# srndpty/kobato-eyes

Measured on AMD Instinct MI355X. Metric: images/s (pHash + all-pairs Hamming scan + cluster membership), higher is better.
Workload: dtype u8 luma, int32 taps (i8 matrix cores), f64 DCT, 1-bit Hamming products (fp4 matrix cores, exact)

## Files before the change

### kobato-eyes_amd/csrc/ke_api.hip

```cpp
#include <cstdarg>
#include <cstdio>
#include <algorithm>
#include <cmath>
#include <numeric>
#include <unordered_map>

#include <fcntl.h>
#include <sys/stat.h>
#include <unistd.h>

#include "ke_internal.h"

static thread_local std::string g_create_err;

int ke_fail(ke_ctx *ctx, int code, const char *fmt, ...) {
    char msg[512];
    va_list ap;
    va_start(ap, fmt);
    vsnprintf(msg, sizeof msg, fmt, ap);
    va_end(ap);
    if (ctx)
        ctx->err = msg;
    else
        g_create_err = msg;
// ... 45 lines not shown
    if (bytes) KE_HIP(ctx, hipMemcpyAsync(d, p, bytes, hipMemcpyHostToDevice, ctx->stream));
    *dev = d;
    return KE_OK;
}

static int upload_i32(ke_ctx *ctx, const std::vector<int32_t> &v, int32_t **out) {
    KE_HIP(ctx, hipMalloc((void **)out, std::max<size_t>(v.size(), 4) * sizeof(int32_t)));
    if (!v.empty())
        KE_HIP(ctx, hipMemcpy(*out, v.data(), v.size() * sizeof(int32_t), hipMemcpyHostToDevice));
    return KE_OK;
}

constexpr size_t kMaxCoeffTables = 2048;

static void free_coeff_cache(ke_ctx *ctx) {
    for (auto &kv : ctx->coeffs) {
        KeAxisCoeffs *c = kv.second;
        for (int32_t *p : {c->d_bounds, c->d_kk, c->d_start, c->d_bias, c->d_packed})
            if (p) (void)hipFree(p);
        for (auto &ck : c->chunked) {
            if (ck.second->d_cstart) (void)hipFree(ck.second->d_cstart);
            if (ck.second->d_cpacked) (void)hipFree(ck.second->d_cpacked);
            if (ck.second->d_cxor) (void)hipFree(ck.second->d_cxor);
            delete ck.second;
        }
        for (auto &mk : c->mx) {
            if (mk.second->d_frag) (void)hipFree(mk.second->d_frag);
            delete mk.second;
        }
        delete c;
    }
    ctx->coeffs.clear();
}

static void trim_coeff_cache(ke_ctx *ctx) {
    if (ctx->coeffs.size() <= kMaxCoeffTables) return;
    (void)hipStreamSynchronize(ctx->stream);
    free_coeff_cache(ctx);
}

const KeAxisCoeffs *ke_get_coeffs(ke_ctx *ctx, int in_size, int out_size, int filter, float in0, float in1) {
    if (in1 < 0.0f) { in0 = 0.0f; in1 = (float)in_size; }
    uint32_t b0, b1;
    std::memcpy(&b0, &in0, 4);
    std::memcpy(&b1, &in1, 4);
    auto key = std::make_tuple(in_size, out_size * 4 + filter, b0, b1);
    auto it = ctx->coeffs.find(key);
    if (it != ctx->coeffs.end()) return it->second;
    auto *c = new KeAxisCoeffs();
    ke_build_axis_coeffs(in_size, out_size, *c, filter, in0, in1);
    if (upload_i32(ctx, c->bounds, &c->d_bounds) || upload_i32(ctx, c->kk, &c->d_kk) ||
        upload_i32(ctx, c->start, &c->d_start) || upload_i32(ctx, c->bias, &c->d_bias) ||
        upload_i32(ctx, c->packed, &c->d_packed)) {
        delete c;
        return nullptr;
    }
    ctx->coeffs[key] = c;
    return c;
}

const KeChunkTable *ke_get_chunks(ke_ctx *ctx, const KeAxisCoeffs *cc, int cpo, int ndwc_multiple) {
    auto *c = const_cast<KeAxisCoeffs *>(cc);
    const int key = cpo * 64 + ndwc_multiple;
    auto it = c->chunked.find(key);
    if (it != c->chunked.end()) return it->second;
    auto *t = new KeChunkTable();
    ke_build_chunked(*c, cpo, *t, ndwc_multiple);
    if (upload_i32(ctx, t->cstart, &t->d_cstart) || upload_i32(ctx, t->cpacked, &t->d_cpacked) ||
        upload_i32(ctx, t->cxor, &t->d_cxor)) {
        delete t;
        return nullptr;
    }
    c->chunked[key] = t;
    return t;
}

const KeMxTable *ke_get_mx(ke_ctx *ctx, const KeAxisCoeffs *cc, int min_ks, bool align64) {
    auto *c = const_cast<KeAxisCoeffs *>(cc);
    const int key = min_ks * 2 + (align64 ? 1 : 0);
    auto it = c->mx.find(key);
    if (it != c->mx.end()) return it->second;
    auto *t = new KeMxTable();
    ke_build_mx(*c, *t, min_ks, align64);
    if (upload_i32(ctx, t->frag, &t->d_frag)) {
        delete t;
        return nullptr;
    }
    c->mx[key] = t;
    return t;
}

void ke_time_begin(ke_ctx *ctx, int kind) {
    ctx->ev_valid[kind] = false;
    (void)hipEventRecord(ctx->ev0[kind], ctx->stream);
}

void ke_time_end(ke_ctx *ctx, int kind) {
    if (hipEventRecord(ctx->ev1[kind], ctx->stream) == hipSuccess) ctx->ev_valid[kind] = true;
}

KE_API int ke_abi_version(void) { return KE_ABI_VERSION; }

KE_API const char *ke_create_error(void) { return g_create_err.c_str(); }

KE_API ke_ctx *ke_create(int device_id) {
    int count = 0;
    if (hipGetDeviceCount(&count) != hipSuccess || count <= 0) {
        ke_fail(nullptr, KE_ENODEV, "no HIP device visible (libkeyes_hip has no CPU fallback)");
        return nullptr;
    }
    if (device_id < 0 || device_id >= count) {
        ke_fail(nullptr, KE_EINVAL, "device_id %d out of range [0,%d)", device_id, count);
        return nullptr;
    }
    if (hipSetDevice(device_id) != hipSuccess) {
        ke_fail(nullptr, KE_EHIP, "hipSetDevice(%d) failed", device_id);
        return nullptr;
    }
    hipDeviceProp_t prop;
    if (hipGetDeviceProperties(&prop, device_id) != hipSuccess) {
        ke_fail(nullptr, KE_EHIP, "hipGetDeviceProperties failed");
        return nullptr;
    }
    if (std::strncmp(prop.gcnArchName, "gfx950", 6) != 0) {
        ke_fail(nullptr, KE_ENODEV, "device %d is %s; this library is built for gfx950 only", device_id,
                prop.gcnArchName);
        return nullptr;
    }
    auto *ctx = new ke_ctx();
    ctx->device = device_id;
    ctx->cu_count = prop.multiProcessorCount;
    if (hipStreamCreateWithFlags(&ctx->own_stream, hipStreamNonBlocking) != hipSuccess) {
        ke_fail(nullptr, KE_EHIP, "hipStreamCreate failed");
        delete ctx;
        return nullptr;
    }
    ctx->stream = ctx->own_stream;
    for (int k = 0; k < KE_T_COUNT; ++k) {
        (void)hipEventCreate(&ctx->ev0[k]);
        (void)hipEventCreate(&ctx->ev1[k]);
    }
    return ctx;
}

static void stage_free(ke_ctx *ctx);

KE_API void ke_destroy(ke_ctx *ctx) {
    if (!ctx) return;
    (void)hipSetDevice(ctx->device);
    (void)hipStreamSynchronize(ctx->stream);
    stage_free(ctx);
    for (int k = 0; k < 2; ++k) {
        if (ctx->side[k]) (void)hipStreamDestroy(ctx->side[k]);
        if (ctx->side_join[k]) (void)hipEventDestroy(ctx->side_join[k]);
    }
    if (ctx->side_fork) (void)hipEventDestroy(ctx->side_fork);
    if (ctx->h_comm) (void)hipHostFree(ctx->h_comm);
    if (ctx->h_meta) (void)hipHostFree(ctx->h_meta);
    for (auto &b : ctx->buf)
        if (b.ptr) (void)hipFree(b.ptr);
    free_coeff_cache(ctx);
    for (int k = 0; k < KE_T_COUNT; ++k) {
        (void)hipEventDestroy(ctx->ev0[k]);
        (void)hipEventDestroy(ctx->ev1[k]);
    }
    (void)hipStreamDestroy(ctx->own_stream);
// ... 982 lines not shown
```

### kobato-eyes_amd/csrc/ke_coeffs.cpp

```cpp
#include <algorithm>
#include <cmath>

#include "ke_internal.h"

namespace {

constexpr int kPrecisionBits = 22;
constexpr double kPi = 3.14159265358979323846;

inline double sinc_pi(double x) {
    if (x == 0.0) return 1.0;
    const double a = x * kPi;
    return std::sin(a) / a;
}

inline double lanczos3(double x) {
    return (x >= -3.0 && x < 3.0) ? sinc_pi(x) * sinc_pi(x / 3.0) : 0.0;
}

inline double triangle(double x) {
    if (x < 0.0) x = -x;
    return x < 1.0 ? 1.0 - x : 0.0;
}

// ... 44 lines not shown
                const double v = total != 0.0 ? w[t] / total : w[t];
                k[t] = v < 0 ? (int32_t)(v * (double)(1 << kPrecisionBits) - 0.5)
                             : (int32_t)(v * (double)(1 << kPrecisionBits) + 0.5);
            }
            c.bounds[2 * o] = lo;
            c.bounds[2 * o + 1] = cnt;
        }
    }

    int ndw = 0;
    c.start.assign((size_t)out_size, 0);
    for (int o = 0; o < out_size; ++o) {
        const int lo = c.bounds[2 * o], cnt = c.bounds[2 * o + 1];
        const int st = lo & ~7;
        c.start[o] = st;
        const int need = (lo + cnt - st + 3) / 4;
        if (need > ndw) ndw = need;
    }
    ndw = (ndw + 3) & ~3;
    c.ndw = ndw;
    c.span = 0;
    c.bias.assign((size_t)out_size, 0);
    c.packed.assign((size_t)out_size * ndw * 3, 0);
    for (int o = 0; o < out_size; ++o) {
        const int lo = c.bounds[2 * o], cnt = c.bounds[2 * o + 1], st = c.start[o];
        if (st + 4 * ndw > c.span) c.span = st + 4 * ndw;
        int64_t ksum = 0;
        for (int j = 0; j < ndw; ++j) {
            uint32_t plane[3] = {0, 0, 0};
            for (int e = 0; e < 4; ++e) {
                const int t = st + 4 * j + e - lo;
                const int32_t k = (t >= 0 && t < cnt) ? c.kk[(size_t)o * c.ksize + t] : 0;
                ksum += k;
                const int32_t b0 = ((k + 128) & 255) - 128;
                const int32_t r1 = (k - b0) >> 8;
                const int32_t b1 = ((r1 + 128) & 255) - 128;
                const int32_t b2 = (r1 - b1) >> 8;
                plane[0] |= (uint32_t)(b0 & 255) << (8 * e);
                plane[1] |= (uint32_t)(b1 & 255) << (8 * e);
                plane[2] |= (uint32_t)(b2 & 255) << (8 * e);
            }
            for (int p = 0; p < 3; ++p) c.packed[((size_t)o * ndw + j) * 3 + p] = (int32_t)plane[p];
        }
        c.bias[o] = (int32_t)(128 * ksum + (1 << (kPrecisionBits - 1)));
    }
}

void ke_build_mx(const KeAxisCoeffs &c, KeMxTable &t, int min_ks, bool align64) {
    t.tiles = (c.out_size + 15) / 16;
    t.base.assign((size_t)t.tiles, 0);
    t.ks = std::max(1, min_ks);
    for (int j = 0; j < t.tiles; ++j) {
        int lo = c.in_size, hi = 0;
        for (int o = 16 * j; o < std::min(16 * j + 16, c.out_size); ++o) {
            lo = std::min(lo, c.bounds[2 * o]);
            hi = std::max(hi, c.bounds[2 * o] + c.bounds[2 * o + 1]);
        }
        const int ks16 = (hi - (lo & ~15) + 63) / 64, ks64 = (hi - (lo & ~63) + 63) / 64;
        t.base[j] = (align64 || ks64 == ks16) ? (lo & ~63) : (lo & ~15);
        t.ks = std::max(t.ks, align64 ? ks64 : ks16);
    }
    t.frag.assign((size_t)t.tiles * t.ks * 3 * 64 * 4, 0);
    for (int j = 0; j < t.tiles; ++j)
        for (int s = 0; s < t.ks; ++s)
            for (int l = 0; l < 64; ++l) {
                const int o = 16 * j + (l & 15);
                if (o >= c.out_size) continue;
                const int lo = c.bounds[2 * o], cnt = c.bounds[2 * o + 1];
                for (int e = 0; e < 16; ++e) {
                    const int tap = t.base[j] + 64 * s + 16 * (l >> 4) + e - lo;
                    const int32_t k = (tap >= 0 && tap < cnt) ? c.kk[(size_t)o * c.ksize + tap] : 0;
                    const int32_t b0 = ((k + 128) & 255) - 128;
                    const int32_t r1 = (k - b0) >> 8;
                    const int32_t b1 = ((r1 + 128) & 255) - 128;
                    const int32_t b2 = (r1 - b1) >> 8;
                    const int32_t plane[3] = {b0, b1, b2};
                    for (int p = 0; p < 3; ++p)
                        t.frag[((((size_t)j * t.ks + s) * 3 + p) * 64 + l) * 4 + e / 4] |=
                            (int32_t)((uint32_t)(plane[p] & 255) << (8 * (e % 4)));
                }
            }
}

void ke_build_chunked(const KeAxisCoeffs &c, int cpo, KeChunkTable &t, int ndwc_multiple) {
    t.cpo = cpo;
    t.ndwc = (((c.ndw + cpo - 1) / cpo) + ndwc_multiple - 1) / ndwc_multiple * ndwc_multiple;
    const int nv = c.out_size * cpo;
    t.cstart.assign((size_t)nv, 0);
    t.cpacked.assign((size_t)nv * t.ndwc * 3, 0);
    t.cspan = 0;
    for (int o = 0; o < c.out_size; ++o)
        for (int k = 0; k < cpo; ++k) {
            const int v = o * cpo + k;
            t.cstart[v] = c.start[o] + 4 * t.ndwc * k;
            if (t.cstart[v] + 4 * t.ndwc > t.cspan) t.cspan = t.cstart[v] + 4 * t.ndwc;
            for (int j = 0; j < t.ndwc; ++j) {
                const int src = k * t.ndwc + j;
                if (src >= c.ndw) continue;
                for (int p = 0; p < 3; ++p)
                    t.cpacked[((size_t)v * t.ndwc + j) * 3 + p] = c.packed[((size_t)o * c.ndw + src) * 3 + p];
            }
        }
    t.cxor.assign((size_t)nv, 0);
    if (t.ndwc % 8 == 0) {
        const int np = t.ndwc / 2;
        for (int g0 = 0; g0 < nv; g0 += 32) {
            for (int v = g0; v < std::min(nv, g0 + 32); ++v) {
                int best_x = 0, best_hits = 1 << 30;
                for (int x = 0; x < 4; ++x) {
                    int hits = 0;
                    for (int p = 0; p < np; ++p) {
                        const int slot = ((t.cstart[v] / 8) + (p ^ x)) & 31;
                        for (int u = g0; u < v; ++u)
                            if ((((t.cstart[u] / 8) + (p ^ t.cxor[u])) & 31) == slot) ++hits;
                    }
                    if (hits < best_hits) { best_hits = hits; best_x = x; }
                }
                t.cxor[v] = best_x;
            }
        }
    }
}
```

### kobato-eyes_amd/csrc/ke_hash.hip

```cpp
#include <cstdlib>

#include "ke_internal.h"
#include "dct_table.h"

namespace {

constexpr int kPrecisionBits = 22;

__device__ __forceinline__ int clip8_fixed(int acc) {
    int v = acc >> kPrecisionBits;
    return v < 0 ? 0 : (v > 255 ? 255 : v);
}

__device__ __forceinline__ int luma_of(const uint8_t *p, int ch) {
    if (ch == 1) return p[0];
    return (int)((19595u * p[0] + 38470u * p[1] + 7471u * p[2] + 0x8000u) >> 16);
}

template <int AXIS>
__global__ __launch_bounds__(256) void ke_resample_pass(const uint8_t *__restrict__ src,
                                                         const uint64_t *__restrict__ offsets, uint64_t stride,
                                                         int ch, int w, int h, const int32_t *__restrict__ bounds,
                                                         const int32_t *__restrict__ kk, int ksize, int out_size,
                                                         uint8_t *__restrict__ dst, int blocks_per_image) {
    const int64_t img = blockIdx.x / blocks_per_image;
    const int blk = blockIdx.x % blocks_per_image;
    const int ow = AXIS == 0 ? out_size : w;
    const int oh = AXIS == 0 ? h : out_size;
    const int e = blk * 256 + threadIdx.x;
    if (e >= ow * oh) return;
    const int oy = e / ow, ox = e % ow;
    const uint8_t *base = src + (offsets ? offsets[img] : (uint64_t)img * stride);
    const int o = AXIS == 0 ? ox : oy;
    const int first = bounds[2 * o], cnt = bounds[2 * o + 1];
    const int32_t *k = kk + (size_t)o * ksize;
    int acc = 1 << (kPrecisionBits - 1);
    if (AXIS == 0) {
        const uint8_t *row = base + ((size_t)oy * w + first) * ch;
        for (int t = 0; t < cnt; ++t) acc += luma_of(row + (size_t)t * ch, ch) * k[t];
    } else {
        const uint8_t *col = base + ((size_t)first * w + ox) * ch;
        for (int t = 0; t < cnt; ++t) acc += luma_of(col + (size_t)t * w * ch, ch) * k[t];
    }
    dst[(size_t)img * ow * oh + e] = (uint8_t)clip8_fixed(acc);
}

__constant__ double c_C32[4][16];
__constant__ double c_C16[2][8];
__constant__ double c_C8[4];

__device__ double dct32_one(const double *x, int k) {
    if (k & 1) {
        const int q = k >> 1;
        double acc = 0.0;
#pragma unroll
        for (int n = 0; n < 16; ++n) acc = fma(x[n] - x[31 - n], c_C32[q][n], acc);
        return acc;
    }
    double u[16];
#pragma unroll
    for (int n = 0; n < 16; ++n) u[n] = x[n] + x[31 - n];
    if (k & 2) {
        const int q = k >> 2;
        double acc = 0.0;
#pragma unroll
        for (int n = 0; n < 8; ++n) acc = fma(u[n] - u[15 - n], c_C16[q][n], acc);
        return acc;
    }
    double v[8];
#pragma unroll
    for (int n = 0; n < 8; ++n) v[n] = u[n] + u[15 - n];
    if (k == 4) {
        double acc = 0.0;
#pragma unroll
        for (int n = 0; n < 4; ++n) acc = fma(v[n] - v[7 - n], c_C8[n], acc);
        return acc;
    }
    const double w0 = v[0] + v[7], w1 = v[1] + v[6], w2 = v[2] + v[5], w3 = v[3] + v[4];
    return (w0 + w1) + (w2 + w3);
}

__device__ uint64_t tile32_to_phash(const uint8_t *tile, double *Td, float *cf, int tid, float *margin = nullptr) {
    {
// ... 160 lines not shown
#pragma unroll
            for (int m = 0; m < 4; ++m) {
                const uint2 v = *reinterpret_cast<const uint2 *>(
                    __builtin_assume_aligned(HT + (size_t)(og + 8 * m) * a.hp + vst + 4 * jj, 8));
                acc[m][0] = __builtin_amdgcn_sdot4((int)v.x, c00, acc[m][0], false);
                acc[m][1] = __builtin_amdgcn_sdot4((int)v.x, c01, acc[m][1], false);
                acc[m][2] = __builtin_amdgcn_sdot4((int)v.x, c02, acc[m][2], false);
                acc[m][0] = __builtin_amdgcn_sdot4((int)v.y, c10, acc[m][0], false);
                acc[m][1] = __builtin_amdgcn_sdot4((int)v.y, c11, acc[m][1], false);
                acc[m][2] = __builtin_amdgcn_sdot4((int)v.y, c12, acc[m][2], false);
            }
        }
        const int vbias = a.v_bias[yy];
#pragma unroll
        for (int m = 0; m < 4; ++m)
            T32[yy * 32 + og + 8 * m] = (uint8_t)clip8_fixed(combine_planes(acc[m][0], acc[m][1], acc[m][2], vbias));
    }
    __syncthreads();
    if (a.tile32_out)
        reinterpret_cast<uint32_t *>(a.tile32_out + (size_t)img * 1024)[tid] = reinterpret_cast<const uint32_t *>(T32)[tid];
    const int64_t slot = a.out_idx ? a.out_idx[img] : img;
    const uint64_t hv = tile32_to_phash(T32, Td, cf, tid, (a.margin && a.phash) ? a.margin + slot : nullptr);
    if (tid == 0 && a.phash) a.phash[slot] = hv;
    if (NDWD > 0) {
        __syncthreads();
        int *part = reinterpret_cast<int *>(Lt);
        uint8_t *T98 = Lt + 1024;
        if (tid < 216) {
            const int out = tid / 3, chunk = tid % 3;
            const int yy = out / 9, oc = out % 9;
            const int vc = yy * 3 + chunk;
            const int vst = a.vd_cstart[vc];
            const int nd = a.ndwcv;
            int d0 = 0, d1 = 0, d2 = 0;
            for (int j = 0; j < nd; j += 2) {
                const int32_t *cp = a.vd_cpacked + ((size_t)vc * nd + j) * 3;
                const uint2 v = *reinterpret_cast<const uint2 *>(__builtin_assume_aligned(HTd + (size_t)oc * a.hpd + vst + 4 * j, 8));
                d0 = __builtin_amdgcn_sdot4((int)v.x, cp[0], d0, false);
                d1 = __builtin_amdgcn_sdot4((int)v.x, cp[1], d1, false);
                d2 = __builtin_amdgcn_sdot4((int)v.x, cp[2], d2, false);
                d0 = __builtin_amdgcn_sdot4((int)v.y, cp[3], d0, false);
                d1 = __builtin_amdgcn_sdot4((int)v.y, cp[4], d1, false);
                d2 = __builtin_amdgcn_sdot4((int)v.y, cp[5], d2, false);
            }
            part[tid] = combine_planes(d0, d1, d2, 0);
        }
        __syncthreads();
        if (tid < 72) {
            const int yy = tid / 9;
            const uint32_t sum = (uint32_t)part[3 * tid] + (uint32_t)part[3 * tid + 1] + (uint32_t)part[3 * tid + 2] + (uint32_t)a.vd_bias[yy];
            T98[tid] = (uint8_t)clip8_fixed((int)sum);
        }
        __syncthreads();
        if (a.tile98_out && tid < 72) a.tile98_out[(size_t)img * 72 + tid] = T98[tid];
        if (tid < 64) {
            const int r = tid >> 3, c = tid & 7;
            const unsigned long long m = __ballot(T98[r * 9 + c + 1] > T98[r * 9 + c]);
            if (tid == 0 && a.dhash) a.dhash[a.out_idx ? a.out_idx[img] : img] = __brevll(m);
        }
    }
}

int upload_dct_tables(ke_ctx *ctx) {
    if (ctx->dct_tables_ready) return KE_OK;
    KE_HIP(ctx, hipMemcpyToSymbol(HIP_SYMBOL(c_C32), KE_C32, sizeof(KE_C32)));
    KE_HIP(ctx, hipMemcpyToSymbol(HIP_SYMBOL(c_C16), KE_C16, sizeof(KE_C16)));
    KE_HIP(ctx, hipMemcpyToSymbol(HIP_SYMBOL(c_C8), KE_C8, sizeof(KE_C8)));
    ctx->dct_tables_ready = true;
    return KE_OK;
}

constexpr int kRTM = 32;
typedef int ke_v4i __attribute__((ext_vector_type(4)));

template <int W64, int KS, bool DH, bool GEN, int C, bool UNAL>
__global__ __launch_bounds__(256, 2) void ke_phash_fused_mx(const KeFusedArgs a) {
    static_assert(!UNAL || GEN, "rows that are not a multiple of 4 pixels need the run-time row length");
    constexpr uint32_t QB = 4u * C;
    constexpr int W = 64 * W64;
    constexpr int QPT = kRTM * (W / 4) / 256;
    const int QW = GEN ? a.qw : W / 4;
    const int QUADS_PER_TILE = kRTM * QW;
    const int LP = GEN ? a.lp : W + 16;
    constexpr int KD = (W64 + 1) / 2;
    extern __shared__ __attribute__((aligned(16))) uint8_t smem[];
    uint8_t *Lt = smem;
    uint8_t *HT = smem + a.lt_bytes;
    uint8_t *HTd = HT + 32 * a.hp;
    uint8_t *X = smem + a.x_off;
    const int tid = threadIdx.x;
    const int lane = tid & 63, wv = tid >> 6;
    const int64_t img = a.bands ? blockIdx.x / a.bands : blockIdx.x;
    const int y_begin = a.bands ? (int)(blockIdx.x % a.bands) * a.band_rows : 0;
    const uint32_t row_bytes = UNAL ? (uint32_t)a.row_bytes : (uint32_t)QW * QB;
    const uint8_t *src = a.pixels + (a.offsets ? a.offsets[img] : (uint64_t)img * a.stride) + (size_t)y_begin * row_bytes;
    const int h = a.bands ? min(a.band_rows, a.h - y_begin) : a.h;
    const uint32_t image_bytes = (uint32_t)(a.h - y_begin) * row_bytes;

    const int mt = wv >> 1, jt = wv & 1;
    ke_v4i bf[KS][3];
#pragma unroll
    for (int s = 0; s < KS; ++s)
#pragma unroll
        for (int p = 0; p < 3; ++p)
            bf[s][p] = reinterpret_cast<const ke_v4i *>(a.mx_frag)[((jt * KS + s) * 3 + p) * 64 + lane];
    constexpr int KDR = DH ? KD : 1;
    ke_v4i bd[KDR][3];
    int dbias = 0;
    if (DH) {
#pragma unroll
        for (int d = 0; d < KDR; ++d)
#pragma unroll
            for (int p = 0; p < 3; ++p)
                bd[d][p] = reinterpret_cast<const ke_v4i *>(a.mxd_frag)[((jt * KD + d) * 3 + p) * 64 + lane];
        dbias = a.hd_bias[(lane & 15) < 9 ? (lane & 15) : 8];
    }
    const int ocol = 16 * jt + (lane & 15);
    const int hbias = a.h_bias[ocol];
    const int a_off = (16 * mt + (lane & 15)) * LP + (jt ? a.mx_base1 : a.mx_base0) + 16 * (lane >> 4);
    const int d_off = (16 * mt + (lane & 15)) * LP + 64 * KD * jt + 16 * (lane >> 4);
    uint8_t *ht_dst = HT + (size_t)ocol * a.hp + 16 * mt + 4 * (lane >> 4);
    uint8_t *htd_dst = HTd + (size_t)(lane & 15) * a.hpd + 16 * mt + 4 * (lane >> 4);
    ke_v4i *x_slot = reinterpret_cast<ke_v4i *>(X + mt * 1024 + lane * 16);

    uint32_t raw[QPT][C];
    auto load_tile = [&](int t) {
        const uint32_t tile_off = UNAL ? (uint32_t)t * (kRTM * row_bytes) : (uint32_t)t * ((uint32_t)QUADS_PER_TILE * QB);
        const uint8_t *tile_ptr = src + tile_off;
        const uint32_t lim = UNAL ? image_bytes - QB - tile_off : min(image_bytes - QB - tile_off, (uint32_t)(QUADS_PER_TILE - 1) * QB);
#pragma unroll
        for (int q = 0; q < QPT; ++q) {
            uint32_t vo = (uint32_t)(q * 256 + tid) * QB;
            if (UNAL) {
                const uint32_t i = min((uint32_t)(q * 256 + tid), (uint32_t)(QUADS_PER_TILE - 1));
                const uint32_t row = __umulhi(i, (uint32_t)a.qw_inv);
                vo = row * row_bytes + (i - row * (uint32_t)QW) * QB;
            }
            const uint32_t off = vo < lim ? vo : lim;
            const uint32_t *p = reinterpret_cast<const uint32_t *>(tile_ptr + off);
#pragma unroll
            for (int k = 0; k < C; ++k) raw[q][k] = __builtin_nontemporal_load(p + k);
        }
    };
    auto store_luma = [&](uint8_t *dst) {
#pragma unroll
        for (int q = 0; q < QPT; ++q) {
            const int i = q * 256 + tid;
            if (GEN) {
                const int row = (int)__umulhi((uint32_t)i, (uint32_t)a.qw_inv);
                if (i < QUADS_PER_TILE)
                    *reinterpret_cast<uint32_t *>(dst + row * LP + (i - row * QW) * 4) = luma4_generic<C>(raw[q]);
            } else {
                *reinterpret_cast<uint32_t *>(dst + (i / (W / 4)) * LP + (i % (W / 4)) * 4) = luma4_generic<C>(raw[q]);
            }
        }
    };
    auto pack_rows = [](const ke_v4i &v0, const ke_v4i &v1, const ke_v4i &v2, int bias) {
        uint32_t packed = 0;
#pragma unroll
        for (int i = 0; i < 4; ++i) packed |= (uint32_t)clip8_fixed(combine_planes(v0[i], v1[i], v2[i], bias)) << (8 * i);
        return packed ^ 0x80808080u;
    };
    auto products = [&](int t, const uint8_t *cur) -> ke_v4i {
        ke_v4i acc[3], dacc[3];
#pragma unroll
        for (int p = 0; p < 3; ++p) acc[p] = dacc[p] = ke_v4i{0, 0, 0, 0};
        const uint8_t *ap = cur + a_off;
#pragma unroll
        for (int s = 0; s < KS; ++s) {
            const ke_v4i av = *reinterpret_cast<const ke_v4i *>(__builtin_assume_aligned(ap + 64 * s, 16));
#pragma unroll
            for (int p = 0; p < 3; ++p) acc[p] = __builtin_amdgcn_mfma_i32_16x16x64_i8(av, bf[s][p], acc[p], 0, 0, 0);
        }
        if (DH) {
            const uint8_t *dp = cur + d_off;
#pragma unroll
            for (int d = 0; d < KDR; ++d) {
                const ke_v4i av = *reinterpret_cast<const ke_v4i *>(__builtin_assume_aligned(dp + 64 * d, 16));
#pragma unroll
                for (int p = 0; p < 3; ++p) dacc[p] = __builtin_amdgcn_mfma_i32_16x16x64_i8(av, bd[d][p], dacc[p], 0, 0, 0);
            }
        }
        *reinterpret_cast<uint32_t *>(ht_dst + t * kRTM) = pack_rows(acc[0], acc[1], acc[2], hbias);
        ke_v4i part;
#pragma unroll
        for (int i = 0; i < 4; ++i) part[i] = combine_planes(dacc[0][i], dacc[1][i], dacc[2][i], 0);
        return part;
    };
    ke_v4i carry = {0, 0, 0, 0};
    auto finish_dhash = [&](int t) {
        const ke_v4i other = x_slot[(t & 1) * 128];
        const ke_v4i zero = {0, 0, 0, 0};
        const ke_v4i sum = carry + other;
        const uint32_t packed = pack_rows(sum, zero, zero, dbias);
        if ((lane & 15) < 9) *reinterpret_cast<uint32_t *>(htd_dst + t * kRTM) = packed;
    };
    auto hpass = [&](int t, const uint8_t *cur) {
        if (!DH) {
            products(t, cur);
        } else if (jt) {
            x_slot[(t & 1) * 128] = products(t, cur);
        } else {
            if (t > 0) finish_dhash(t - 1);
            carry = products(t, cur);
        }
    };

    const int ntiles = (h + kRTM - 1) / kRTM;
    load_tile(0);
    store_luma(Lt);
    __syncthreads();
    for (int t = 0; t + 1 < ntiles; ++t) {
        load_tile(t + 1);
        __builtin_amdgcn_sched_barrier(0);
        hpass(t, Lt + (t & 1) * a.lt_half);
        __builtin_amdgcn_sched_barrier(0);
        store_luma(Lt + ((t + 1) & 1) * a.lt_half);
        __syncthreads();
    }
    if (UNAL) {
        if (tid == 0 && y_begin + h == a.h)
            patch_last_quad<C>(src + (size_t)(h - 1) * row_bytes, a.w, Lt + ((ntiles - 1) & 1) * a.lt_half + ((h - 1) - (ntiles - 1) * kRTM) * LP);
        __syncthreads();
    }
    hpass(ntiles - 1, Lt + ((ntiles - 1) & 1) * a.lt_half);
    __syncthreads();
    if (DH) {
        if (!jt) finish_dhash(ntiles - 1);
        __syncthreads();
    }
    if (a.bands) {
        band_writeout(HT, a.hp, 32, h, a.hs + (size_t)img * 32 * a.hs_hp + y_begin, a.hs_hp, tid, 256);
        if (DH) band_writeout(HTd, a.hpd, 9, h, a.hsd + (size_t)img * 9 * a.hsd_hp + y_begin, a.hsd_hp, tid, 256);
        return;
    }
    fused_tail<(DH ? 1 : 0)>(a, Lt, HT, HTd, tid, img);
}

struct KeBandPlan {
    int bands, band_rows;
    uint8_t *hs, *hsd;
    int hs_hp, hsd_hp;
};

template <int W64, int KS, bool DH, bool GEN = false, int C = 3, bool UNAL = false>
int launch_fused_mx(ke_ctx *ctx, const KeHashGroup &g, const KeAxisCoeffs *ch, const KeAxisCoeffs *cv, uint64_t *d_phash,
                    uint8_t *d_tile32, uint64_t *d_dhash, uint8_t *d_tile98, const KeBandPlan *plan = nullptr) {
    const int W = g.w;
    if (GEN ? (W > 64 * W64 || W <= 64 * (W64 - 1) || (W % 4 != 0) != UNAL) : W != 64 * W64) return KE_EUNSUPPORTED;
    const KeMxTable *mx = ke_get_mx(ctx, ch, KS);
    if (!mx) return ke_fail(ctx, KE_EHIP, "coefficient upload failed");
    if (mx->tiles != 2 || mx->ks != KS) return KE_EUNSUPPORTED;
    KeFusedArgs a;
    std::memset(&a, 0, sizeof a);
    a.pixels = g.pixels; a.offsets = g.offsets; a.stride = g.stride; a.out_idx = g.out_idx; a.h = g.h;
    a.h_bias = ch->d_bias;
    a.v_packed = cv->d_packed; a.v_start = cv->d_start; a.v_bias = cv->d_bias;
    a.ndwv = cv->ndw;
    a.mx_frag = mx->d_frag; a.mx_base0 = mx->base[0]; a.mx_base1 = mx->base[1];
    const int rows_padded = plan ? plan->band_rows : ((g.h + kRTM - 1) / kRTM) * kRTM;
    if (plan) { a.bands = plan->bands; a.band_rows = plan->band_rows; a.hs = plan->hs; a.hsd = plan->hsd; a.hs_hp = plan->hs_hp; a.hsd_hp = plan->hsd_hp; }
    constexpr int KD = (W64 + 1) / 2;
    const int overhang = std::max(0, std::max(std::max(mx->base[0], mx->base[1]) + 64 * KS, DH ? 128 * KD : 0) - W);
    a.qw = (W + 3) / 4;
    a.w = W; a.row_bytes = W * C;
    a.qw_inv = (int)(uint32_t)((0x100000000ull + (uint64_t)a.qw - 1) / (uint64_t)a.qw);
    a.lp = GEN ? (((W + 15) / 16 + 1) | 1) * 16 : W + 16;
    a.lt_half = (kRTM * a.lp + overhang + 15) & ~15;
    a.lt_bytes = 2 * a.lt_half;
    a.hp = ((std::max(plan ? 0 : cv->span, rows_padded) + 7) & ~7) + 8;
    a.hpd = 8;
    a.phash = d_phash; a.tile32_out = d_tile32; a.margin = ctx->margin_cur;
    size_t lds = std::max<size_t>((size_t)a.lt_bytes + (size_t)32 * a.hp, 4096);
    if (DH) {
        const KeAxisCoeffs *chd = ke_get_coeffs(ctx, g.w, 9), *cvd = ke_get_coeffs(ctx, g.h, 8);
        if (!chd || !cvd) return ke_fail(ctx, KE_EHIP, "coefficient upload failed");
        const KeMxTable *mxd = ke_get_mx(ctx, chd, 2 * KD);
        const KeChunkTable *tv = ke_get_chunks(ctx, cvd, 3);
        if (!mxd || !tv) return ke_fail(ctx, KE_EHIP, "coefficient upload failed");
        if (mxd->tiles != 1 || mxd->base[0] != 0 || mxd->ks != 2 * KD) return KE_EUNSUPPORTED;
        a.mxd_frag = mxd->d_frag;
        a.hd_bias = chd->d_bias;
        a.vd_cpacked = tv->d_cpacked; a.vd_cstart = tv->d_cstart; a.vd_bias = cvd->d_bias;
        a.ndwcv = tv->ndwc;
        a.hpd = ((std::max(plan ? 0 : tv->cspan, rows_padded) + 7) & ~7) + 8;
        a.dhash = d_dhash; a.tile98_out = d_tile98;
        lds += (size_t)9 * a.hpd;
        lds = (lds + 15) & ~(size_t)15;
        a.x_off = (int)lds;
        lds += 4096;
    }
    if (lds > 150 * 1024) return KE_EUNSUPPORTED;
    if (!plan && lds > 80 * 1024 && lds - (size_t)(32 * (a.hp - 136)) - (DH ? (size_t)(9 * (a.hpd - 136)) : 0) <= 80 * 1024) return KE_EUNSUPPORTED;
    if (lds > 64 * 1024)
        KE_HIP(ctx, hipFuncSetAttribute(reinterpret_cast<const void *>(&ke_phash_fused_mx<W64, KS, DH, GEN, C, UNAL>),
                                        hipFuncAttributeMaxDynamicSharedMemorySize, (int)lds));
    if (g.n * (plan ? plan->bands : 1) > 0x7fffffffLL) return ke_fail(ctx, KE_EUNSUPPORTED, "group too large for one launch");
    hipLaunchKernelGGL((ke_phash_fused_mx<W64, KS, DH, GEN, C, UNAL>), dim3((unsigned)(g.n * (plan ? plan->bands : 1))), dim3(256), lds, ctx->stream, a);
    KE_HIP(ctx, hipGetLastError());
    return KE_OK;
}

constexpr int kRTW = 16;

template <int KSH, int QPT, bool DH, int KDW, int C, bool UNAL>
__global__ __launch_bounds__(512, 1) void ke_phash_fused_wide(const KeFusedArgs a) {
    constexpr uint32_t QB = 4u * C;
    extern __shared__ __attribute__((aligned(16))) uint8_t smem[];
    uint8_t *Lt = smem;
    uint8_t *HT = smem + a.lt_bytes;
    uint8_t *HTd = HT + 32 * a.hp;
    uint8_t *X = smem + a.x_off;
    const int tid = threadIdx.x;
    const int lane = tid & 63, wv = tid >> 6;
    const int jt = wv & 1, kh = wv >> 1;
    const int64_t img = a.bands ? blockIdx.x / a.bands : blockIdx.x;
    const int y_begin = a.bands ? (int)(blockIdx.x % a.bands) * a.band_rows : 0;
    const int QW = a.qw, LP = a.lp;
    const uint32_t row_bytes = UNAL ? (uint32_t)a.row_bytes : (uint32_t)QW * QB;
    const uint8_t *src = a.pixels + (a.offsets ? a.offsets[img] : (uint64_t)img * a.stride) + (size_t)y_begin * row_bytes;
    const int h = a.bands ? min(a.band_rows, a.h - y_begin) : a.h;
    const int quads_per_tile = kRTW * QW;
    const uint32_t image_bytes = (uint32_t)(a.h - y_begin) * row_bytes;

    ke_v4i bf[KSH][3];
#pragma unroll
    for (int s = 0; s < KSH; ++s)
#pragma unroll
        for (int p = 0; p < 3; ++p)
            bf[s][p] = reinterpret_cast<const ke_v4i *>(a.mx_frag)[((jt * 4 * KSH + kh * KSH + s) * 3 + p) * 64 + lane];
    const int ocol = 16 * jt + (lane & 15);
    const int hbias = a.h_bias[ocol];
    const int a_off = (lane & 15) * LP + (jt ? a.mx_base1 : a.mx_base0) + 64 * KSH * kh + 16 * (lane >> 4);
    uint8_t *ht_dst = HT + (size_t)ocol * a.hp + 4 * (lane >> 4);
    ke_v4i *x_slot = reinterpret_cast<ke_v4i *>(X) + jt * 192 + lane;
    constexpr int KDR = DH ? KDW : 1;
    ke_v4i bd[KDR][3];
    int dbias = 0;
    if (DH) {
#pragma unroll
        for (int d = 0; d < KDR; ++d)
#pragma unroll
            for (int p = 0; p < 3; ++p)
                bd[d][p] = reinterpret_cast<const ke_v4i *>(a.mxd_frag)[((wv * KDW + d) * 3 + p) * 64 + lane];
        dbias = a.hd_bias[(lane & 15) < 9 ? (lane & 15) : 8];
    }
    const int d_off = (lane & 15) * LP + 64 * KDW * wv + 16 * (lane >> 4);
    uint8_t *htd_dst = HTd + (size_t)(lane & 15) * a.hpd + 4 * (lane >> 4);
    ke_v4i *xd_slot = reinterpret_cast<ke_v4i *>(X) + 768 + lane;

    uint32_t raw[QPT][C];
    auto load_tile = [&](int t) {
        const uint32_t tile_off = UNAL ? (uint32_t)t * (kRTW * row_bytes) : (uint32_t)t * ((uint32_t)quads_per_tile * QB);
        const uint8_t *tile_ptr = src + tile_off;
        const uint32_t lim = UNAL ? image_bytes - QB - tile_off : min(image_bytes - QB - tile_off, (uint32_t)(quads_per_tile - 1) * QB);
#pragma unroll
        for (int q = 0; q < QPT; ++q) {
            uint32_t vo = (uint32_t)(q * 512 + tid) * QB;
            if (UNAL) {
                const uint32_t i = min((uint32_t)(q * 512 + tid), (uint32_t)(quads_per_tile - 1));
                const uint32_t row = __umulhi(i, (uint32_t)a.qw_inv);
                vo = row * row_bytes + (i - row * (uint32_t)QW) * QB;
            }
            const uint32_t off = vo < lim ? vo : lim;
            const uint32_t *p = reinterpret_cast<const uint32_t *>(tile_ptr + off);
#pragma unroll
            for (int c = 0; c < C; ++c) raw[q][c] = __builtin_nontemporal_load(p + c);
        }
    };
    auto store_luma = [&](uint8_t *dst) {
#pragma unroll
        for (int q = 0; q < QPT; ++q) {
            const int i = q * 512 + tid;
// ... 1077 lines not shown
```

### kobato-eyes_amd/csrc/ke_internal.h

```cpp
#pragma once

#include <hip/hip_runtime.h>

#include <cstdint>
#include <cstring>
#include <map>
#include <string>
#include <thread>
#include <tuple>
#include <utility>
#include <vector>

#include "../../include/keyes.h"

#define KE_API extern "C" __attribute__((visibility("default")))

struct KeAxisCoeffs {
    int in_size = 0, out_size = 0;
    int ksize = 0;
    std::vector<int32_t> bounds;
    std::vector<int32_t> kk;
    int ndw = 0;
    int span = 0;
    std::vector<int32_t> start;
    std::vector<int32_t> bias;
    std::vector<int32_t> packed;
    int32_t *d_bounds = nullptr, *d_kk = nullptr, *d_start = nullptr, *d_bias = nullptr, *d_packed = nullptr;
    std::map<int, struct KeChunkTable *> chunked;
    std::map<int, struct KeMxTable *> mx;
};

struct KeMxTable {
    int tiles = 0, ks = 0;
    std::vector<int32_t> base;
    std::vector<int32_t> frag;
    int32_t *d_frag = nullptr;
};

struct KeChunkTable {
    int cpo = 0, ndwc = 0, cspan = 0;
    std::vector<int32_t> cstart, cpacked;
    std::vector<int32_t> cxor;
    int32_t *d_cstart = nullptr, *d_cpacked = nullptr, *d_cxor = nullptr;
};


void ke_build_axis_coeffs(int in_size, int out_size, KeAxisCoeffs &out, int filter, float in0, float in1);
void ke_build_chunked(const KeAxisCoeffs &c, int cpo, KeChunkTable &out, int ndwc_multiple = 4);
void ke_build_mx(const KeAxisCoeffs &c, KeMxTable &out, int min_ks = 0, bool align64 = false);

struct KeDevBuf {
    void *ptr = nullptr;
    size_t bytes = 0;
};

enum { KE_T_HASH = 0, KE_T_SCAN = 1, KE_T_SSIM = 2, KE_T_SYNTH = 3, KE_T_JPEG = 4, KE_T_COUNT = 5 };
enum {
    KE_BUF_PIXELS = 0,
    KE_BUF_TMP,
    KE_BUF_TILE32,
    KE_BUF_TILE98,
    KE_BUF_OUT0,
    KE_BUF_OUT1,
    KE_BUF_OUT2,
    KE_BUF_META,
    KE_BUF_SCAN_IN,
    KE_BUF_SCAN_AUX,
    KE_BUF_SCAN_EDGES,
    KE_BUF_SCAN_CNT,
    KE_BUF_SCAN_HIST,
    KE_BUF_SCAN_EXP,
    KE_BUF_SSIM_IN,
    KE_BUF_SSIM_AUX,
    KE_BUF_COMM,
    KE_BUF_COMM_EDGES,
    KE_BUF_JPEG_TABLES,
    KE_BUF_COUNT
};

constexpr int KE_MAX_STAGE_SLOTS = 4;
struct KeStageSlot {
    uint8_t *h_px = nullptr, *d_px = nullptr;
    uint64_t *h_meta = nullptr, *d_meta = nullptr;
    uint64_t *h_ph = nullptr, *h_dh = nullptr, *d_ph = nullptr, *d_dh = nullptr;
    float *h_mg = nullptr, *d_mg = nullptr;
    hipEvent_t copied = nullptr, done = nullptr;
    bool in_flight = false;
    bool px_external = false;
    uint64_t *user_ph = nullptr, *user_dh = nullptr;
    float *user_mg = nullptr;
    int64_t n = 0;
};
struct KeStage {
    size_t bytes = 0;
    int64_t max_images = 0;
    int n_slots = 0, next = 0;
    hipStream_t copy_stream = nullptr;
    KeStageSlot slot[KE_MAX_STAGE_SLOTS];
};

struct ke_ctx {
    int device = 0;
    int cu_count = 0;
    hipStream_t own_stream = nullptr;
    hipStream_t stream = nullptr;
    std::string err;
    KeDevBuf buf[KE_BUF_COUNT];
    std::map<std::tuple<int, int, uint32_t, uint32_t>, KeAxisCoeffs *> coeffs;
    hipEvent_t ev0[KE_T_COUNT] = {}, ev1[KE_T_COUNT] = {};
    bool ev_valid[KE_T_COUNT] = {};
    KeStage *stage = nullptr;
    hipStream_t side[2] = {nullptr, nullptr};
    hipEvent_t side_fork = nullptr, side_join[2] = {nullptr, nullptr};
    int64_t edge_slots = 1024;
    void *h_comm = nullptr;
    size_t h_comm_bytes = 0;
    void *h_meta = nullptr;
    size_t h_meta_bytes = 0;
    bool ssim_exact = false;
    float *margin_cur = nullptr;
    bool dct_tables_ready = false;
};

int ke_fail(ke_ctx *ctx, int code, const char *fmt, ...);
#define KE_HIP(ctx, call)                                                                        \
    do {                                                                                         \
        hipError_t e_ = (call);                                                                  \
        if (e_ != hipSuccess)                                                                    \
            return ke_fail((ctx), KE_EHIP, "%s failed: %s (%s:%d)", #call, hipGetErrorString(e_), \
                           __FILE__, __LINE__);                                                  \
    } while (0)
#define KE_TRY(expr)            \
    do {                        \
        int rc_ = (expr);       \
        if (rc_ != KE_OK) return rc_; \
    } while (0)

bool ke_is_device_ptr(const void *p);
int ke_reserve(ke_ctx *ctx, int which, size_t bytes, void **out);
int ke_to_device(ke_ctx *ctx, const void *p, size_t bytes, int which, const void **dev);
const KeAxisCoeffs *ke_get_coeffs(ke_ctx *ctx, int in_size, int out_size, int filter = KE_FILTER_LANCZOS, float in0 = 0.0f,
                                  float in1 = -1.0f);
const KeChunkTable *ke_get_chunks(ke_ctx *ctx, const KeAxisCoeffs *c, int cpo, int ndwc_multiple = 4);
const KeMxTable *ke_get_mx(ke_ctx *ctx, const KeAxisCoeffs *c, int min_ks = 0, bool align64 = false);
void ke_time_begin(ke_ctx *ctx, int kind);
void ke_time_end(ke_ctx *ctx, int kind);

struct KeHashGroup {
    const uint8_t *pixels;
    const uint64_t *offsets;
    uint64_t stride;
    const int64_t *out_idx;
    int64_t n;
    int w, h, channels;
    bool misaligned = false;
};
int ke_launch_hash_group(ke_ctx *ctx, const KeHashGroup &g, uint64_t *d_phash, uint64_t *d_dhash,
                         uint8_t *d_tile32_out, uint8_t *d_tile98_out, hipStream_t fused_stream = nullptr);
int ke_launch_resize_group(ke_ctx *ctx, const KeHashGroup &g, int ow, int oh, int filter, uint8_t *d_tiles,
                           const float *box = nullptr);
int ke_launch_tile_ahash(ke_ctx *ctx, const uint8_t *d_tiles, int64_t n, int grid, int tile, uint64_t *d_bits);
int ke_launch_sad_pairs(ke_ctx *ctx, const uint8_t *d_thumbs, int64_t pixels, const int64_t *d_pa, const int64_t *d_pb,
                        int64_t n_pairs, uint64_t *d_out);
int ke_launch_band_pairs_after_size(ke_ctx *ctx, const uint64_t *d_hashes, const int64_t *d_sizes, int64_t n, int band_bits,
                                    int band_count, double ratio, int64_t bucket_pair_cap, unsigned long long *d_out);
int ke_launch_scan(ke_ctx *ctx, const uint64_t *d_hashes, const int64_t *d_ids, const int64_t *d_sizes, int64_t n,
                   int part_index, int part_count, int threshold, int band_bits, int band_count, double size_ratio,
                   int64_t bucket_pair_cap, ke_edge *d_edges, int64_t capacity, unsigned long long *d_counters,
                   unsigned long long *pairs_evaluated, bool want_bucket_pairs);
int ke_launch_ssim(ke_ctx *ctx, const uint8_t *d_images, int w, int h, int channels, const int64_t *d_pa,
                   const int64_t *d_pb, int64_t n_pairs, double *d_out);
int ke_launch_synth_rgb(ke_ctx *ctx, uint64_t seed, int64_t first, const int64_t *d_indices, int64_t n, int w, int h,
                        uint8_t *d_out);
int ke_launch_synth_hashes(ke_ctx *ctx, uint64_t seed, int64_t n, uint64_t *d_out);

template <typename Fn>
static inline int ke_parallel_ranges(int64_t n, Fn fn) {
    int want = (int)std::thread::hardware_concurrency();
    if (const char *e = std::getenv("KE_HOST_THREADS")) want = std::atoi(e);
    int nt = (int)std::min<int64_t>(std::max(want, 1), std::min<int64_t>(16, n / 256));
    if (nt <= 1) { fn((int64_t)0, n, 0); return 1; }
    std::vector<std::thread> th;
    for (int t = 0; t < nt; ++t) th.emplace_back([=]() { fn(n * t / nt, n * (t + 1) / nt, t); });
    for (auto &x : th) x.join();
    return nt;
}
```

Baseline: 8.654 million.

## Pack dHash byte planes into MFMA columns and share A-fragment loads with pHash

The dHash horizontal pass now puts the three byte planes of the 9-output filter into the columns of a single 16x16 MFMA tile (5 outputs per plane), split across the two column tiles. The planes are then recombined with DPP lane shifts instead of running three separate MFMA accumulators and exchanging K-halves through shared memory. In the non-generic path, the pHash horizontal products reuse the A operands already loaded for dHash. This removes duplicate LDS loads, the LDS exchange buffer and an extra barrier. In exchange, the path now requires specific base alignments (otherwise it returns unsupported), and each wave issues MFMAs over the full width instead of half of it.

```diff
diff --git a/kobato-eyes_amd/csrc/ke_api.hip b/kobato-eyes_amd/csrc/ke_api.hip
--- a/kobato-eyes_amd/csrc/ke_api.hip
+++ b/kobato-eyes_amd/csrc/ke_api.hip
@@ -151,6 +151,21 @@
     if (it != c->mx.end()) return it->second;
     auto *t = new KeMxTable();
     ke_build_mx(*c, *t, min_ks, align64);
+    if (upload_i32(ctx, t->frag, &t->d_frag)) {
+        delete t;
+        return nullptr;
+    }
+    c->mx[key] = t;
+    return t;
+}
+
+const KeMxTable *ke_get_mx_planes(ke_ctx *ctx, const KeAxisCoeffs *cc, int ks) {
+    auto *c = const_cast<KeAxisCoeffs *>(cc);
+    const int key = -ks;
+    auto it = c->mx.find(key);
+    if (it != c->mx.end()) return it->second;
+    auto *t = new KeMxTable();
+    ke_build_mx_planes(*c, *t, ks);
     if (upload_i32(ctx, t->frag, &t->d_frag)) {
         delete t;
         return nullptr;
diff --git a/kobato-eyes_amd/csrc/ke_coeffs.cpp b/kobato-eyes_amd/csrc/ke_coeffs.cpp
--- a/kobato-eyes_amd/csrc/ke_coeffs.cpp
+++ b/kobato-eyes_amd/csrc/ke_coeffs.cpp
@@ -150,6 +150,30 @@
             }
 }
 
+void ke_build_mx_planes(const KeAxisCoeffs &c, KeMxTable &t, int ks) {
+    t.tiles = 2;
+    t.base.assign(2, 0);
+    t.ks = ks;
+    t.frag.assign((size_t)2 * ks * 64 * 4, 0);
+    for (int j = 0; j < 2; ++j)
+        for (int s = 0; s < ks; ++s)
+            for (int l = 0; l < 64; ++l) {
+                const int n = l & 15, p = n / kMxPlaneOutputs, o = kMxPlaneOutputs * j + n % kMxPlaneOutputs;
+                if (p >= 3 || o >= c.out_size) continue;
+                const int lo = c.bounds[2 * o], cnt = c.bounds[2 * o + 1];
+                for (int e = 0; e < 16; ++e) {
+                    const int tap = 64 * s + 16 * (l >> 4) + e - lo;
+                    const int32_t k = (tap >= 0 && tap < cnt) ? c.kk[(size_t)o * c.ksize + tap] : 0;
+                    const int32_t b0 = ((k + 128) & 255) - 128;
+                    const int32_t r1 = (k - b0) >> 8;
+                    const int32_t b1 = ((r1 + 128) & 255) - 128;
+                    const int32_t b2 = (r1 - b1) >> 8;
+                    const int32_t plane[3] = {b0, b1, b2};
+                    t.frag[(((size_t)j * ks + s) * 64 + l) * 4 + e / 4] |= (int32_t)((uint32_t)(plane[p] & 255) << (8 * (e % 4)));
+                }
+            }
+}
+
 void ke_build_chunked(const KeAxisCoeffs &c, int cpo, KeChunkTable &t, int ndwc_multiple) {
     t.cpo = cpo;
     t.ndwc = (((c.ndw + cpo - 1) / cpo) + ndwc_multiple - 1) / ndwc_multiple * ndwc_multiple;
diff --git a/kobato-eyes_amd/csrc/ke_hash.hip b/kobato-eyes_amd/csrc/ke_hash.hip
--- a/kobato-eyes_amd/csrc/ke_hash.hip
+++ b/kobato-eyes_amd/csrc/ke_hash.hip
@@ -1,4 +1,5 @@
 #include <cstdlib>
+#include <type_traits>
 
 #include "ke_internal.h"
 #include "dct_table.h"
@@ -325,12 +326,11 @@
     const int QW = GEN ? a.qw : W / 4;
     const int QUADS_PER_TILE = kRTM * QW;
     const int LP = GEN ? a.lp : W + 16;
-    constexpr int KD = (W64 + 1) / 2;
+    constexpr bool SHARE = DH && !GEN;
     extern __shared__ __attribute__((aligned(16))) uint8_t smem[];
     uint8_t *Lt = smem;
     uint8_t *HT = smem + a.lt_bytes;
     uint8_t *HTd = HT + 32 * a.hp;
-    uint8_t *X = smem + a.x_off;
     const int tid = threadIdx.x;
     const int lane = tid & 63, wv = tid >> 6;
     const int64_t img = a.bands ? blockIdx.x / a.bands : blockIdx.x;
@@ -347,24 +347,22 @@
 #pragma unroll
         for (int p = 0; p < 3; ++p)
             bf[s][p] = reinterpret_cast<const ke_v4i *>(a.mx_frag)[((jt * KS + s) * 3 + p) * 64 + lane];
-    constexpr int KDR = DH ? KD : 1;
-    ke_v4i bd[KDR][3];
+    constexpr int KDR = DH ? W64 : 1;
+    ke_v4i bd[KDR];
     int dbias = 0;
+    const bool d_valid = DH && (lane & 15) < (jt ? 9 - kMxPlaneOutputs : kMxPlaneOutputs);
+    const int dcol = d_valid ? kMxPlaneOutputs * jt + (lane & 15) : 0;
     if (DH) {
 #pragma unroll
-        for (int d = 0; d < KDR; ++d)
-#pragma unroll
-            for (int p = 0; p < 3; ++p)
-                bd[d][p] = reinterpret_cast<const ke_v4i *>(a.mxd_frag)[((jt * KD + d) * 3 + p) * 64 + lane];
-        dbias = a.hd_bias[(lane & 15) < 9 ? (lane & 15) : 8];
+        for (int d = 0; d < KDR; ++d) bd[d] = reinterpret_cast<const ke_v4i *>(a.mxd_frag)[(jt * W64 + d) * 64 + lane];
+        dbias = a.hd_bias[dcol];
     }
     const int ocol = 16 * jt + (lane & 15);
     const int hbias = a.h_bias[ocol];
     const int a_off = (16 * mt + (lane & 15)) * LP + (jt ? a.mx_base1 : a.mx_base0) + 16 * (lane >> 4);
-    const int d_off = (16 * mt + (lane & 15)) * LP + 64 * KD * jt + 16 * (lane >> 4);
+    const int d_off = (16 * mt + (lane & 15)) * LP + 16 * (lane >> 4);
     uint8_t *ht_dst = HT + (size_t)ocol * a.hp + 16 * mt + 4 * (lane >> 4);
-    uint8_t *htd_dst = HTd + (size_t)(lane & 15) * a.hpd + 16 * mt + 4 * (lane >> 4);
-    ke_v4i *x_slot = reinterpret_cast<ke_v4i *>(X + mt * 1024 + lane * 16);
+    uint8_t *htd_dst = HTd + (size_t)dcol * a.hpd + 16 * mt + 4 * (lane >> 4);
 
     uint32_t raw[QPT][C];
     auto load_tile = [&](int t) {
@@ -404,49 +402,61 @@
         for (int i = 0; i < 4; ++i) packed |= (uint32_t)clip8_fixed(combine_planes(v0[i], v1[i], v2[i], bias)) << (8 * i);
         return packed ^ 0x80808080u;
     };
-    auto products = [&](int t, const uint8_t *cur) -> ke_v4i {
-        ke_v4i acc[3], dacc[3];
-#pragma unroll
-        for (int p = 0; p < 3; ++p) acc[p] = dacc[p] = ke_v4i{0, 0, 0, 0};
-        const uint8_t *ap = cur + a_off;
-#pragma unroll
-        for (int s = 0; s < KS; ++s) {
-            const ke_v4i av = *reinterpret_cast<const ke_v4i *>(__builtin_assume_aligned(ap + 64 * s, 16));
-#pragma unroll
-            for (int p = 0; p < 3; ++p) acc[p] = __builtin_amdgcn_mfma_i32_16x16x64_i8(av, bf[s][p], acc[p], 0, 0, 0);
-        }
-        if (DH) {
+    auto store_dhash = [&](int t, const ke_v4i &dacc) {
+        ke_v4i d1, d2;
+#pragma unroll
+        for (int i = 0; i < 4; ++i) {
+            d1[i] = __builtin_amdgcn_update_dpp(0, dacc[i], 0x100 + kMxPlaneOutputs, 0xf, 0xf, true);
+            d2[i] = __builtin_amdgcn_update_dpp(0, dacc[i], 0x100 + 2 * kMxPlaneOutputs, 0xf, 0xf, true);
+        }
+        uint32_t packed = 0;
+#pragma unroll
+        for (int i = 0; i < 4; ++i) {
+            int v = combine_planes(dacc[i], d1[i], d2[i], dbias) >> kPrecisionBits;
+            asm("" : "+v"(v));
+            packed |= (uint32_t)(v < 0 ? 0 : (v > 255 ? 255 : v)) << (8 * i);
+        }
+        if (d_valid) *reinterpret_cast<uint32_t *>(htd_dst + t * kRTM) = packed ^ 0x80808080u;
+    };
+    auto products = [&](int t, const uint8_t *cur, auto JT) {
+        ke_v4i acc[3], dacc = {0, 0, 0, 0};
+#pragma unroll
+        for (int p = 0; p < 3; ++p) acc[p] = ke_v4i{0, 0, 0, 0};
+        if (SHARE) {
+            constexpr int SB = decltype(JT)::value ? W64 - KS : 0;
             const uint8_t *dp = cur + d_off;
 #pragma unroll
             for (int d = 0; d < KDR; ++d) {
                 const ke_v4i av = *reinterpret_cast<const ke_v4i *>(__builtin_assume_aligned(dp + 64 * d, 16));
-#pragma unroll
-                for (int p = 0; p < 3; ++p) dacc[p] = __builtin_amdgcn_mfma_i32_16x16x64_i8(av, bd[d][p], dacc[p], 0, 0, 0);
+                if (d >= SB && d < SB + KS) {
+#pragma unroll
+                    for (int p = 0; p < 3; ++p) acc[p] = __builtin_amdgcn_mfma_i32_16x16x64_i8(av, bf[d - SB][p], acc[p], 0, 0, 0);
+                }
+                dacc = __builtin_amdgcn_mfma_i32_16x16x64_i8(av, bd[d], dacc, 0, 0, 0);
+            }
+        } else {
+            const uint8_t *ap = cur + a_off;
+#pragma unroll
+            for (int s = 0; s < KS; ++s) {
+                const ke_v4i av = *reinterpret_cast<const ke_v4i *>(__builtin_assume_aligned(ap + 64 * s, 16));
+#pragma unroll
+                for (int p = 0; p < 3; ++p) acc[p] = __builtin_amdgcn_mfma_i32_16x16x64_i8(av, bf[s][p], acc[p], 0, 0, 0);
+            }
+            if (DH) {
+                const uint8_t *dp = cur + d_off;
+#pragma unroll
+                for (int d = 0; d < KDR; ++d) {
+                    const ke_v4i av = *reinterpret_cast<const ke_v4i *>(__builtin_assume_aligned(dp + 64 * d, 16));
+                    dacc = __builtin_amdgcn_mfma_i32_16x16x64_i8(av, bd[d], dacc, 0, 0, 0);
+                }
             }
         }
         *reinterpret_cast<uint32_t *>(ht_dst + t * kRTM) = pack_rows(acc[0], acc[1], acc[2], hbias);
-        ke_v4i part;
-#pragma unroll
-        for (int i = 0; i < 4; ++i) part[i] = combine_planes(dacc[0][i], dacc[1][i], dacc[2][i], 0);
-        return part;
-    };
-    ke_v4i carry = {0, 0, 0, 0};
-    auto finish_dhash = [&](int t) {
-        const ke_v4i other = x_slot[(t & 1) * 128];
-        const ke_v4i zero = {0, 0, 0, 0};
-        const ke_v4i sum = carry + other;
-        const uint32_t packed = pack_rows(sum, zero, zero, dbias);
-        if ((lane & 15) < 9) *reinterpret_cast<uint32_t *>(htd_dst + t * kRTM) = packed;
+        if (DH) store_dhash(t, dacc);
     };
     auto hpass = [&](int t, const uint8_t *cur) {
-        if (!DH) {
-            products(t, cur);
-        } else if (jt) {
-            x_slot[(t & 1) * 128] = products(t, cur);
-        } else {
-            if (t > 0) finish_dhash(t - 1);
-            carry = products(t, cur);
-        }
+        if (SHARE && jt) products(t, cur, std::integral_constant<int, 1>{});
+        else products(t, cur, std::integral_constant<int, 0>{});
     };
 
     const int ntiles = (h + kRTM - 1) / kRTM;
@@ -468,10 +478,6 @@
     }
     hpass(ntiles - 1, Lt + ((ntiles - 1) & 1) * a.lt_half);
     __syncthreads();
-    if (DH) {
-        if (!jt) finish_dhash(ntiles - 1);
-        __syncthreads();
-    }
     if (a.bands) {
         band_writeout(HT, a.hp, 32, h, a.hs + (size_t)img * 32 * a.hs_hp + y_begin, a.hs_hp, tid, 256);
         if (DH) band_writeout(HTd, a.hpd, 9, h, a.hsd + (size_t)img * 9 * a.hsd_hp + y_begin, a.hsd_hp, tid, 256);
@@ -503,8 +509,7 @@
     a.mx_frag = mx->d_frag; a.mx_base0 = mx->base[0]; a.mx_base1 = mx->base[1];
     const int rows_padded = plan ? plan->band_rows : ((g.h + kRTM - 1) / kRTM) * kRTM;
     if (plan) { a.bands = plan->bands; a.band_rows = plan->band_rows; a.hs = plan->hs; a.hsd = plan->hsd; a.hs_hp = plan->hs_hp; a.hsd_hp = plan->hsd_hp; }
-    constexpr int KD = (W64 + 1) / 2;
-    const int overhang = std::max(0, std::max(std::max(mx->base[0], mx->base[1]) + 64 * KS, DH ? 128 * KD : 0) - W);
+    const int overhang = std::max(0, std::max(std::max(mx->base[0], mx->base[1]) + 64 * KS, DH ? 64 * W64 : 0) - W);
     a.qw = (W + 3) / 4;
     a.w = W; a.row_bytes = W * C;
     a.qw_inv = (int)(uint32_t)((0x100000000ull + (uint64_t)a.qw - 1) / (uint64_t)a.qw);
@@ -518,10 +523,10 @@
     if (DH) {
         const KeAxisCoeffs *chd = ke_get_coeffs(ctx, g.w, 9), *cvd = ke_get_coeffs(ctx, g.h, 8);
         if (!chd || !cvd) return ke_fail(ctx, KE_EHIP, "coefficient upload failed");
-        const KeMxTable *mxd = ke_get_mx(ctx, chd, 2 * KD);
+        const KeMxTable *mxd = ke_get_mx_planes(ctx, chd, W64);
         const KeChunkTable *tv = ke_get_chunks(ctx, cvd, 3);
         if (!mxd || !tv) return ke_fail(ctx, KE_EHIP, "coefficient upload failed");
-        if (mxd->tiles != 1 || mxd->base[0] != 0 || mxd->ks != 2 * KD) return KE_EUNSUPPORTED;
+        if (!GEN && (mx->base[0] != 0 || mx->base[1] != 64 * (W64 - KS))) return KE_EUNSUPPORTED;
         a.mxd_frag = mxd->d_frag;
         a.hd_bias = chd->d_bias;
         a.vd_cpacked = tv->d_cpacked; a.vd_cstart = tv->d_cstart; a.vd_bias = cvd->d_bias;
@@ -530,8 +535,6 @@
         a.dhash = d_dhash; a.tile98_out = d_tile98;
         lds += (size_t)9 * a.hpd;
         lds = (lds + 15) & ~(size_t)15;
-        a.x_off = (int)lds;
-        lds += 4096;
     }
     if (lds > 150 * 1024) return KE_EUNSUPPORTED;
     if (!plan && lds > 80 * 1024 && lds - (size_t)(32 * (a.hp - 136)) - (DH ? (size_t)(9 * (a.hpd - 136)) : 0) <= 80 * 1024) return KE_EUNSUPPORTED;
diff --git a/kobato-eyes_amd/csrc/ke_internal.h b/kobato-eyes_amd/csrc/ke_internal.h
--- a/kobato-eyes_amd/csrc/ke_internal.h
+++ b/kobato-eyes_amd/csrc/ke_internal.h
@@ -48,6 +48,8 @@
 void ke_build_axis_coeffs(int in_size, int out_size, KeAxisCoeffs &out, int filter, float in0, float in1);
 void ke_build_chunked(const KeAxisCoeffs &c, int cpo, KeChunkTable &out, int ndwc_multiple = 4);
 void ke_build_mx(const KeAxisCoeffs &c, KeMxTable &out, int min_ks = 0, bool align64 = false);
+constexpr int kMxPlaneOutputs = 5;
+void ke_build_mx_planes(const KeAxisCoeffs &c, KeMxTable &out, int ks);
 
 struct KeDevBuf {
     void *ptr = nullptr;
@@ -143,6 +145,7 @@
                                   float in1 = -1.0f);
 const KeChunkTable *ke_get_chunks(ke_ctx *ctx, const KeAxisCoeffs *c, int cpo, int ndwc_multiple = 4);
 const KeMxTable *ke_get_mx(ke_ctx *ctx, const KeAxisCoeffs *c, int min_ks = 0, bool align64 = false);
+const KeMxTable *ke_get_mx_planes(ke_ctx *ctx, const KeAxisCoeffs *c, int ks);
 void ke_time_begin(ke_ctx *ctx, int kind);
 void ke_time_end(ke_ctx *ctx, int kind);
 
```

Result: no change. 8.643 million (-0.1%).
